# CMU-SAFARI/AirLift

Hardware: NVIDIA B200
Metric: remapped reads/sec at 1/2/4/8 B200; ksw2 GCUPS; seed-lookup HBM GB/s (higher is better)
Workload: dtype u8/int32

## Files before the change

airlift_b200/csrc/mmg_stages.cu:

```cuda
#include <cub/cub.cuh>
#include "mmg_ctx.cuh"
#include "mmg_regheap.h"
#include "mmg_sketchwarp.h"
#include "mmg_rswarp.h"

int mmg_run_sketch(mmg_ctx_t *c, const uint32_t *d_S, const SketchUnit *d_units, int n_units, int w, int k, int is_hpc,
                   DevBuf &cnt, DevBuf &off, DevBuf &out, int64_t *total, bool short_reads, uint64_t stage_slots);

#define MMG_READ_CHUNK 4096


__global__ void k_encode_reads(const uint8_t *__restrict__ ascii, const uint64_t *__restrict__ seq_off, const int32_t *__restrict__ seq_len,
                               const uint64_t *__restrict__ q_off, const uint8_t *__restrict__ flip, int n_seq, uint64_t n_words,
                               uint32_t *__restrict__ Q)
{
	const uint64_t wi = (uint64_t)blockIdx.x * blockDim.x + threadIdx.x;
	if (wi >= n_words) return;
	const uint64_t b0 = wi * 8;
	int lo = 0, hi = n_seq - 1;
	while (lo < hi) { const int mid = (lo + hi + 1) >> 1; if (q_off[mid] <= b0) lo = mid; else hi = mid - 1; }
	const int r = lo, len = seq_len[r];
	const uint64_t base = b0 - q_off[r];
	const uint8_t *s = ascii + seq_off[r];
	const bool fl = flip[r] != 0;
	uint32_t word = 0;
	for (int j = 0; j < 8; ++j) {
		const uint64_t i = base + j;
// ... 48 lines not shown
			if (n > 0 && n < max_occ) run += n;
		}
	}
	if (replay) {
		const int m = (int)(e - b);
		uint8_t dup = m > 256 ? 1 : 0;
		for (int i = 0; i < m && !dup; ++i) {
			if (m_n[b + i] <= 0 || m_n[b + i] >= max_occ) continue;
			const uint64_t h = mv[b + i].x >> 8;
			for (int j = i + 1; j < m; ++j)
				if (mv[b + j].x >> 8 == h && m_n[b + j] > 0 && m_n[b + j] < max_occ) { dup = 1; break; }
		}
		if (dup) {
			int kept = 0;
			for (int i = 0; i < m; ++i) kept += m_n[b + i] > 0 && m_n[b + i] < max_occ;
			dup = (kept <= 256 && n_a < (1 << 24)) ? 1 : 2;
		}
		replay[li] = dup;
	}
}

__global__ void k_expand(FragTab ft, const int32_t *__restrict__ list, int n_list, const mm128 *__restrict__ mv, const int32_t *__restrict__ m_n,
                         const uint64_t *__restrict__ m_val, const uint64_t *__restrict__ pos, int max_occ, int64_t flag,
                         const int64_t *__restrict__ aoff, const uint8_t *__restrict__ replay, int64_t n_total,
                         uint64_t *__restrict__ key, uint64_t *__restrict__ val, int32_t *__restrict__ n_skipped, const int32_t *__restrict__ m_aoff)
{
	const int64_t g = (int64_t)blockIdx.x * blockDim.x + threadIdx.x;
	if (g >= n_total) return;
	const int li = frag_of_anchor(aoff, n_list, g);
	if (replay[li] == 2) return;
	const int f = list ? list[li] : li;
	const int64_t b = ft.unit_off[ft.unit0[f]], e = ft.unit_off[ft.unit0[f + 1]];
	int64_t i = g - aoff[li];
	int m;
	{
		int lo = 0, hi = (int)(e - b) - 1;
		while (lo < hi) { const int mid = (lo + hi + 1) >> 1; if (m_aoff[b + mid] <= i) lo = mid; else hi = mid - 1; }
		m = lo;
		i -= m_aoff[b + m];
	}
	const mm128 mz = mv[b + m];
	const uint64_t r = mmg_hit_pos(pos, m_n[b + m], m_val[b + m], (uint32_t)i);
	if (replay[li] == 1) { key[g] = r, val[g] = (uint64_t)(g - aoff[li]); return; }
	if (mmg_skip_seed(flag, r, (uint32_t)mz.y)) { key[g] = MMG_NONE, val[g] = 0; atomicAdd(&n_skipped[li], 1); return; }
	const mm128 an = mmg_make_anchor(r, mz, mmg_is_tandem(mv + b, (int)(e - b), m), ft.qlen[f]);
	key[g] = (an.x & (1ULL << 63)) | r;
	val[g] = an.y;
}

__global__ void k_sort_segments(int n_list, const int64_t *__restrict__ aoff, const uint8_t *__restrict__ replay, int64_t *__restrict__ seg_b, int64_t *__restrict__ seg_e)
{
	const int li = blockIdx.x * blockDim.x + threadIdx.x;
	if (li >= n_list) return;
	seg_b[li] = aoff[li];
	seg_e[li] = replay[li] == 2 ? aoff[li] : aoff[li + 1];
}

__global__ void k_emit_sorted(int n_list, const int64_t *__restrict__ aoff, const uint8_t *__restrict__ replay, int64_t n_total,
                              const uint64_t *__restrict__ key, const uint64_t *__restrict__ val, const int32_t *__restrict__ n_skipped,
                              int32_t *__restrict__ na, mm128 *__restrict__ a, uint8_t *__restrict__ tie )
{
	const int64_t g = (int64_t)blockIdx.x * blockDim.x + threadIdx.x;
	if (g >= n_total) return;
	const int li = frag_of_anchor(aoff, n_list, g);
	if (replay[li]) return;
	const uint64_t k = key[g];
	if (g == aoff[li]) na[li] = (int32_t)(aoff[li + 1] - aoff[li]) - n_skipped[li];
	if (k == MMG_NONE) return;
	const uint64_t r = k & ~(1ULL << 63);
	mm128 an;
	an.x = (k & (1ULL << 63)) | (r & 0xffffffff00000000ULL) | ((uint32_t)r >> 1);
	an.y = val[g];
	a[g] = an;
	if (tie && g > aoff[li]) {
		const uint64_t kp = key[g - 1], rp = kp & ~(1ULL << 63);
		if (((kp & (1ULL << 63)) | (rp & 0xffffffff00000000ULL) | ((uint32_t)rp >> 1)) == an.x) tie[li] = 1;
	}
}

__global__ void __launch_bounds__(128)
k_fill_flat_warp(int n_list, const int64_t *__restrict__ aoff, const uint8_t *__restrict__ tie, const uint64_t *__restrict__ key,
                 const uint64_t *__restrict__ val, int32_t *__restrict__ na, mm128 *__restrict__ a, int32_t *__restrict__ work, RsFrame *__restrict__ stack)
{
	__shared__ int32_t s_head[4][256], s_tail[4][256];
	const int li = (int)(((int64_t)blockIdx.x * blockDim.x + threadIdx.x) >> 5), lane = threadIdx.x & 31, wi = threadIdx.x >> 5;
	if (li >= n_list || tie[li] != 1) return;
	const int64_t ao = aoff[li];
	const int32_t n_plan = (int32_t)(aoff[li + 1] - ao);
	mm128 *A = a + ao;
	int32_t o = 0;
	for (int32_t i0 = 0; i0 < n_plan; i0 += 32) {
		const int32_t i = i0 + lane;
		const uint64_t k = i < n_plan ? key[ao + i] : MMG_NONE;
		const unsigned m = __ballot_sync(0xffffffffu, k != MMG_NONE);
		if (k != MMG_NONE) {
			const uint64_t r = k & ~(1ULL << 63);
			mm128 an;
			an.x = (k & (1ULL << 63)) | (r & 0xffffffff00000000ULL) | ((uint32_t)r >> 1);
			an.y = val[ao + i];
			A[o + __popc(m & ((1u << lane) - 1u))] = an;
		}
		o += __popc(m);
	}
	__syncwarp();
	mm128 *tmp = reinterpret_cast<mm128*>(work + ao * 8);
	int32_t *dst = reinterpret_cast<int32_t*>(tmp + n_plan);
	uint8_t *dig = reinterpret_cast<uint8_t*>(dst + n_plan);
	const WarpDev wp = {lane};
	mmg_rs_sort_warp(wp, A, (int64_t)o, tmp, dst, dig, stack + ao / 65 + 2 * (int64_t)li, s_head[wi], s_tail[wi], KeyX());
	if (lane == 0) na[li] = o;
}


__global__ void k_heap_rank(int n_list, const int64_t *__restrict__ aoff, const uint8_t *__restrict__ replay, int64_t n_total,
                            const uint64_t *__restrict__ key, const uint64_t *__restrict__ val, uint32_t *__restrict__ K)
{
	const int64_t g = (int64_t)blockIdx.x * blockDim.x + threadIdx.x;
	if (g >= n_total) return;
	const int li = frag_of_anchor(aoff, n_list, g);
	if (replay[li] != 1) return;
	const int64_t ao = aoff[li];
	int64_t l = g;
	const uint64_t k = key[g];
	while (l > ao && key[l - 1] == k) --l;
	K[ao + (int64_t)val[g]] = (uint32_t)(l - ao);
}

__global__ void k_heap_list(int n_list, const uint8_t *__restrict__ replay, int32_t *__restrict__ out, int32_t *__restrict__ counters)
{
	const int li = blockIdx.x * blockDim.x + threadIdx.x;
	if (li >= n_list) return;
	if (replay[li] == 1) out[atomicAdd(&counters[0], 1)] = li;
	else if (replay[li] == 2) atomicAdd(&counters[2], 1);
}

#define HEAP_MAX_LISTS 256
#define HEAP_RING 16

struct HeapList { int32_t first, cnt, cur, m; };

__device__ __forceinline__ void heap_sift_root(uint32_t *l, uint32_t n, uint32_t tmp, uint32_t *root_out)
{
	uint32_t i = 0, root = tmp;
	const uint32_t INF = 0xffffffffu;
	for (;;) {
		const uint32_t c = 2 * i + 1;
		if (c >= n) break;
		const uint32_t g = 2 * c + 1;
		const uint32_t a = l[c], b = c + 1 < n ? l[c + 1] : INF;
		const uint32_t g0 = g < n ? l[g] : INF, g1 = g + 1 < n ? l[g + 1] : INF, g2 = g + 2 < n ? l[g + 2] : INF, g3 = g + 3 < n ? l[g + 3] : INF;
		const bool right = c + 1 < n && (a >> 8) > (b >> 8);
		const uint32_t k = right ? c + 1 : c, v = right ? b : a;
		if ((v >> 8) > (tmp >> 8)) break;
		l[i] = v;
		if (i == 0) root = v;
		i = k;
		const uint32_t c2 = 2 * k + 1;
// ... 1169 lines not shown
                    int64_t n_mv, int max_occ, const PassBufs &pb, bool want_mini, uint8_t *d_flag, int64_t *n_anchors)
{
	*n_anchors = 0;
	if (n_list == 0) return MMG_OK;
	MMG_TRY(pb.na->ensure((size_t)(n_list + 1) * 4));
	MMG_TRY(pb.aoff->ensure((size_t)(n_list + 1) * 8));
	MMG_TRY(pb.rep->ensure((size_t)(n_list + 1) * 4));
	MMG_TRY(pb.nmini->ensure((size_t)(n_list + 1) * 4));
	MMG_TRY(pb.nu->ensure((size_t)(n_list + 1) * 4));
	MMG_TRY(pb.nv->ensure((size_t)(n_list + 1) * 4));
	if (want_mini) MMG_TRY(pb.mini->ensure((size_t)(n_mv + 1) * 8));
	const bool heap_path = (opt->flag & MMG_F_HEAP_SORT) != 0;
	MMG_TRY(c->d_replay.ensure((size_t)n_list + 16));
	MMG_CUDA(cudaMemsetAsync(pb.na->p, 0, (size_t)(n_list + 1) * 4, c->stream));
	MMG_CUDA(cudaMemsetAsync(pb.nu->p, 0, (size_t)(n_list + 1) * 4, c->stream));
	MMG_CUDA(cudaMemsetAsync(pb.nv->p, 0, (size_t)(n_list + 1) * 4, c->stream));
	MMG_CUDA(cudaMemsetAsync(pb.nmini->p, 0, (size_t)(n_list + 1) * 4, c->stream));
	MMG_LAUNCH(c, k_plan, mmg_blocks(n_list, 128), 128, 0, ft, d_list, n_list, c->d_mv.as<mm128>(), c->d_m_n.as<int32_t>(), max_occ,
	           pb.na->as<int32_t>(), pb.rep->as<int32_t>(), pb.nmini->as<int32_t>(), want_mini ? pb.mini->as<uint64_t>() : nullptr,
	           heap_path ? c->d_replay.as<uint8_t>() : nullptr, c->d_m_aoff.as<int32_t>());
	MMG_TRY(scan_i32_to_i64(c, pb.na->as<int32_t>(), pb.aoff->as<int64_t>(), n_list + 1));
	int32_t *hp_counters = nullptr, *rlist = nullptr, *hp = nullptr;
	if (heap_path) {
		MMG_TRY(c->d_hlist.ensure(((size_t)n_list + 8) * 4));
		MMG_TRY(c->h_path.ensure(64));
		hp_counters = c->d_hlist.as<int32_t>(), rlist = hp_counters + 4, hp = c->h_path.as<int32_t>() + (d_flag ? 0 : 4);
		MMG_CUDA(cudaMemsetAsync(hp_counters, 0, 16, c->stream));
		MMG_LAUNCH(c, k_heap_list, mmg_blocks(n_list, 256), 256, 0, n_list, c->d_replay.as<uint8_t>(), rlist, hp_counters);
		MMG_D2H(c, hp, hp_counters, 16);
	}
	int64_t tot = 0;
	MMG_D2H(c, &tot, pb.aoff->as<int64_t>() + n_list, 8);
	MMG_CUDA(cudaStreamSynchronize(c->stream));
	*n_anchors = tot;
	MMG_TRY(pb.a->ensure((size_t)(tot + 1) * 16));
	MMG_TRY(pb.work->ensure((size_t)(tot + 1) * 32));
	MMG_TRY(pb.u->ensure((size_t)(tot + 1) * 16));
	MMG_TRY(pb.b->ensure((size_t)(tot + 1) * 16));
	MMG_TRY(pb.stack->ensure((size_t)(tot / 65 + 2 * (size_t)n_list + 4) * sizeof(RsFrame)));
	MMG_TRY(c->d_heap.ensure((size_t)(n_mv + 1) * 16));
	uint8_t *d_tie = nullptr;
	if (!heap_path) {
		MMG_TRY(c->d_tie.ensure((size_t)n_list + 16));
		d_tie = c->d_tie.as<uint8_t>();
		MMG_CUDA(cudaMemsetAsync(d_tie, 0, (size_t)n_list + 16, c->stream));
		MMG_CUDA(cudaMemsetAsync(c->d_replay.p, 0, (size_t)n_list + 16, c->stream));
	}
	if (tot > 0) {
		MMG_TRY(c->d_skey.ensure(((size_t)tot + 1) * 16)); MMG_TRY(c->d_sval.ensure(((size_t)tot + 1) * 16));
		MMG_TRY(c->d_sseg.ensure(((size_t)n_list + 1) * 20 + 64));
		uint64_t *k0 = c->d_skey.as<uint64_t>(), *k1 = k0 + tot + 1, *v0 = c->d_sval.as<uint64_t>(), *v1 = v0 + tot + 1;
		int64_t *seg_b = c->d_sseg.as<int64_t>(), *seg_e = seg_b + n_list + 1;
		int32_t *n_skipped = reinterpret_cast<int32_t*>(seg_e + n_list + 1);
		MMG_CUDA(cudaMemsetAsync(n_skipped, 0, (size_t)n_list * 4, c->stream));
		MMG_LAUNCH(c, k_expand, mmg_blocks(tot, 256), 256, 0, ft, d_list, n_list, c->d_mv.as<mm128>(), c->d_m_n.as<int32_t>(), c->d_m_val.as<uint64_t>(),
		           mi->d_pos, max_occ, opt->flag, pb.aoff->as<int64_t>(), c->d_replay.as<uint8_t>(), tot, k0, v0, n_skipped, c->d_m_aoff.as<int32_t>());
		MMG_LAUNCH(c, k_sort_segments, mmg_blocks(n_list, 256), 256, 0, n_list, pb.aoff->as<int64_t>(), c->d_replay.as<uint8_t>(), seg_b, seg_e);
		{
			size_t tmp = 0;
			cub::DeviceSegmentedSort::SortPairs(nullptr, tmp, k0, k1, v0, v1, tot, n_list, seg_b, seg_e, c->stream);
			MMG_TRY(c->d_cub.ensure(tmp));
			MMG_TIMED(c, "cub_segmented_sort(seed hits)", cub::DeviceSegmentedSort::SortPairs(c->d_cub.p, tmp, k0, k1, v0, v1, tot, n_list, seg_b, seg_e, c->stream));
		}
		MMG_LAUNCH(c, k_emit_sorted, mmg_blocks(tot, 256), 256, 0, n_list, pb.aoff->as<int64_t>(), c->d_replay.as<uint8_t>(), tot, k1, v1, n_skipped,
		           pb.na->as<int32_t>(), pb.a->as<mm128>(), d_tie);
	}
	if (heap_path && tot > 0) {
		MMG_TRY(c->d_hrank.ensure(((size_t)tot + 1) * 4));
		MMG_TRY(c->d_hpop.ensure(((size_t)tot + 1) * 4));
		int32_t *counters = hp_counters;
		const uint64_t *k1 = c->d_skey.as<uint64_t>() + tot + 1, *v1 = c->d_sval.as<uint64_t>() + tot + 1;
		if (hp[0] > 0) {
			MMG_LAUNCH(c, k_heap_rank, mmg_blocks(tot, 256), 256, 0, n_list, pb.aoff->as<int64_t>(), c->d_replay.as<uint8_t>(), tot, k1, v1, c->d_hrank.as<uint32_t>());
			MMG_LAUNCH(c, k_heap_replay, hp[0] < 148 * 8 ? hp[0] : 148 * 8, 32, 0, ft, d_list, rlist, counters, c->d_mv.as<mm128>(), c->d_m_n.as<int32_t>(), c->d_m_val.as<uint64_t>(),
			           c->d_m_aoff.as<int32_t>(), mi->d_pos, max_occ, opt->flag, pb.aoff->as<int64_t>(), c->d_hrank.as<uint32_t>(), c->d_hpop.as<uint32_t>());
			MMG_LAUNCH(c, k_heap_emit, hp[0], HEAP_EMIT_THREADS, 0, ft, d_list, rlist, c->d_mv.as<mm128>(), c->d_m_n.as<int32_t>(), c->d_m_val.as<uint64_t>(),
			           c->d_m_aoff.as<int32_t>(), mi->d_pos, max_occ, opt->flag, pb.aoff->as<int64_t>(), c->d_hpop.as<uint32_t>(), pb.na->as<int32_t>(), pb.a->as<mm128>(),
			           c->d_frag_iter.as<unsigned long long>() + 1);
		}
	}
	if (!heap_path) {
		if (tot > 0)
			MMG_LAUNCH(c, k_fill_flat_warp, mmg_blocks((size_t)n_list * 32, 128), 128, 0, n_list, pb.aoff->as<int64_t>(), d_tie, c->d_skey.as<uint64_t>(),
			           c->d_sval.as<uint64_t>(), pb.na->as<int32_t>(), pb.a->as<mm128>(), pb.work->as<int32_t>(), pb.stack->as<RsFrame>());
	} else {
		const int per_warp = d_flag == nullptr || n_list <= 4096 ? 1 : 0;
		MMG_LAUNCH(c, k_fill, mmg_blocks(per_warp ? (size_t)n_list * 32 : (size_t)n_list, 64), 64, 0, ft, d_list, n_list, c->d_mv.as<mm128>(), c->d_m_n.as<int32_t>(),
		           c->d_m_val.as<uint64_t>(), mi->d_pos, max_occ, opt->flag, pb.aoff->as<int64_t>(), pb.na->as<int32_t>(), pb.a->as<mm128>(), c->d_heap.as<mm128>(),
		           pb.stack->as<RsFrame>(), heap_path ? c->d_replay.as<uint8_t>() : d_tie, heap_path ? 2 : 1, per_warp);
	}
	if (getenv("MMG_TRACE")) {
		std::vector<uint8_t> hr((size_t)n_list); std::vector<int32_t> hn((size_t)n_list);
		cudaStreamSynchronize(c->stream);
		cudaMemcpy(hr.data(), heap_path ? c->d_replay.p : (void*)d_tie, (size_t)n_list, cudaMemcpyDeviceToHost);
		cudaMemcpy(hn.data(), pb.na->p, (size_t)n_list * 4, cudaMemcpyDeviceToHost);
		int64_t nr = 0, ar = 0, amax = 0, big = 0, abig = 0, big_all = 0, abig_all = 0;
		for (int i = 0; i < n_list; ++i) {
			if (hn[i] > 4096) ++big_all, abig_all += hn[i];
			if (!hr[i]) continue;
			++nr, ar += hn[i]; if (hn[i] > amax) amax = hn[i]; if (hn[i] > 4096) ++big, abig += hn[i];
		}
		fprintf(stderr, "[mmg::pass] max_occ %d: %d fragments, %lld anchors; > 4096 anchors: %lld fragments with %lld anchors; literal replay: %lld fragments, %lld anchors, largest %lld, "
		        "of which > 4096 anchors: %lld fragments with %lld anchors\n", max_occ, n_list, (long long)tot, (long long)big_all, (long long)abig_all, (long long)nr, (long long)ar, (long long)amax, (long long)big, (long long)abig);
	}
	ChainOptDev co;
	co.bw = opt->bw, co.max_gap = opt->max_gap, co.max_gap_ref = opt->max_gap_ref, co.max_frag_len = opt->max_frag_len;
	co.max_skip = opt->max_chain_skip, co.max_iter = opt->max_chain_iter, co.min_cnt = opt->min_cnt, co.min_sc = opt->min_chain_score;
	co.is_cdna = !!(opt->flag & MMG_F_SPLICE), co.is_sr = !!(opt->flag & MMG_F_SR);
	if (tot > 0) {
		MMG_TRY(c->d_seg_head.ensure((size_t)tot + 16));
		MMG_TRY(c->d_seg_start.ensure(((size_t)tot + 2) * 8 + 64));
		MMG_TRY(c->d_seg_avg.ensure((size_t)(n_list + 1) * 4));
		int64_t *seg_start = c->d_seg_start.as<int64_t>();
		int32_t *d_nseg = reinterpret_cast<int32_t*>(seg_start + tot + 1), *d_next = d_nseg + 1, *d_nlong = d_nseg + 2;
		MMG_CUDA(cudaMemsetAsync(d_nseg, 0, 16, c->stream));
		MMG_TRY(c->d_seg_li.ensure(((size_t)tot + 1) * 4));
		MMG_TRY(c->d_seg_long.ensure(((size_t)tot / CHAIN_SMALL_SEG + 2) * 4));
		MMG_LAUNCH(c, k_chain_heads, mmg_blocks(tot, 256), 256, 0, ft, d_list, n_list, c->d_misc.as<int32_t>(), co, pb.aoff->as<int64_t>(),
		           pb.na->as<int32_t>(), pb.a->as<mm128>(), tot, c->d_seg_head.as<uint8_t>(), pb.work->as<int32_t>(), c->d_seg_li.as<int32_t>());
		MMG_LAUNCH(c, k_chain_avgspan, mmg_blocks((size_t)n_list * 32, 128), 128, 0, n_list, pb.aoff->as<int64_t>(), pb.na->as<int32_t>(),
		           pb.a->as<mm128>(), c->d_seg_avg.as<float>());
		{
			size_t tmp = 0;
			cub::CountingInputIterator<int64_t> it(0);
			cub::DeviceSelect::Flagged(nullptr, tmp, it, c->d_seg_head.as<uint8_t>(), seg_start, d_nseg, tot, c->stream);
			MMG_TRY(c->d_cub.ensure(tmp));
// ... 51 lines not shown
{
	MMG_CUDA(cudaSetDevice(c->dev));
	ResidentBatch &rb = c->rb;
	const int nf = rb.n_frag;
	memset(out, 0, sizeof(*out));
	out->n_frag = nf;
	if (nf == 0) return MMG_OK;
	if (mi->w > MMG_MAX_W) { mmg_set_error("w=%d exceeds the device limit %d", mi->w, MMG_MAX_W); return MMG_ELIMIT; }
	MMG_CUDA(cudaEventRecord(c->ev[0], c->stream));
	int64_t n_mv = 0;
	MMG_TRY(mmg_run_sketch(c, c->d_Q.as<uint32_t>(), c->d_units.as<SketchUnit>(), rb.n_units, mi->w, mi->k, mi->is_hpc, c->d_unit_cnt,
	                       c->d_unit_off, c->d_mv, &n_mv, rb.max_len <= SKW_MAX_LEN, rb.q_words * 8));
	MMG_TRY(c->d_m_n.ensure((size_t)(n_mv + 1) * 4));
	MMG_TRY(c->d_m_val.ensure((size_t)(n_mv + 1) * 8));
	MMG_TRY(c->d_m_aoff.ensure((size_t)(n_mv + 1) * 4));
	if (n_mv) MMG_LAUNCH(c, k_lookup, mmg_blocks(n_mv, 256), 256, 0, mi->view(), c->d_mv.as<mm128>(), n_mv, c->d_m_n.as<int32_t>(), c->d_m_val.as<uint64_t>());
	FragTab ft;
	ft.unit0 = c->d_frag_unit0.as<int32_t>(), ft.unit_off = c->d_unit_off.as<int64_t>(), ft.qlen = c->d_frag_qlen.as<int32_t>();
	const bool want_mini = !(opt->flag & MMG_F_SR);
	MMG_TRY(c->d_frag_flag.ensure((size_t)nf + 16));
	MMG_TRY(c->d_frag_iter.ensure(16));
	MMG_CUDA(cudaMemsetAsync(c->d_frag_flag.p, 0, (size_t)nf + 16, c->stream));
	MMG_CUDA(cudaMemsetAsync(c->d_frag_iter.p, 0, 16, c->stream));
	MMG_TRY(c->h_path.ensure(64));
	memset(c->h_path.p, 0, 64);
	PassBufs p1 = {&c->d_frag_na, &c->d_frag_aoff, &c->d_frag_rep, &c->d_frag_nmini, &c->d_mini, &c->d_a, &c->d_work, &c->d_u, &c->d_b,
	               &c->d_stack, &c->d_frag_nu, &c->d_frag_nv};
	int64_t n_anch1 = 0, n_anch2 = 0;
	MMG_TRY(run_pass(c, mi, opt, ft, nullptr, nf, n_mv, opt->mid_occ, p1, want_mini, c->d_frag_flag.as<uint8_t>(), &n_anch1));
	std::vector<int32_t> list;
	std::vector<uint8_t> hflag(nf);
	MMG_TRY(c->d_frag_list.ensure((size_t)(nf + 1) * 8));
	int32_t *d_list = c->d_frag_list.as<int32_t>(), *d_src = d_list + nf;
	MMG_CUDA(cudaMemsetAsync(d_src, 0xff, (size_t)nf * 4, c->stream));
	if (opt->max_occ > opt->mid_occ) {
		MMG_D2H(c, hflag.data(), c->d_frag_flag.p, nf);
		MMG_CUDA(cudaStreamSynchronize(c->stream));
		for (int f = 0; f < nf; ++f) if (hflag[f]) list.push_back(f);
	}
	PassBufs p2 = {&c->d2_frag_na, &c->d2_frag_aoff, &c->d2_frag_rep, &c->d2_frag_nmini, &c->d2_mini, &c->d2_a, &c->d2_work, &c->d2_u, &c->d2_b,
	               &c->d2_stack, &c->d2_frag_nu, &c->d2_frag_nv};
	const int n2 = (int)list.size();
	if (n2) {
		MMG_H2D(c, d_list, list.data(), (size_t)n2 * 4);
		MMG_TRY(run_pass(c, mi, opt, ft, d_list, n2, n_mv, opt->max_occ, p2, want_mini, nullptr, &n_anch2));
		MMG_LAUNCH(c, k_merge_pass2, mmg_blocks(n2, 128), 128, 0, n2, d_list, c->d2_frag_nu.as<int32_t>(), c->d2_frag_nv.as<int32_t>(),
		           c->d2_frag_rep.as<int32_t>(), c->d2_frag_nmini.as<int32_t>(), c->d_frag_nu.as<int32_t>(), c->d_frag_nv.as<int32_t>(),
		           c->d_frag_rep.as<int32_t>(), c->d_frag_nmini.as<int32_t>(), d_src);
// ... 34 lines not shown
		uint64_t *ho = reinterpret_cast<uint64_t*>(c->h_out_meta.as<uint8_t>() + ((meta_i + 15) & ~(size_t)15));
		MMG_D2H(c, hi, c->d_frag_nu.p, (size_t)nf * 4);
		MMG_D2H(c, hi + nf, c->d_frag_nv.p, (size_t)nf * 4);
		MMG_D2H(c, hi + 2 * nf, c->d_frag_rep.p, (size_t)nf * 4);
		MMG_D2H(c, hi + 3 * nf, c->d_frag_nmini.p, (size_t)nf * 4);
		MMG_D2H(c, hi + 4 * nf, d_src, (size_t)nf * 4);
		MMG_D2H(c, ho, c->d_uoff.p, (size_t)(nf + 1) * 8);
		MMG_D2H(c, ho + (nf + 1), c->d_voff.p, (size_t)(nf + 1) * 8);
		if (want_mini) MMG_D2H(c, ho + 2 * (nf + 1), c->d_moff.p, (size_t)(nf + 1) * 8);
		if (tot[0]) MMG_D2H(c, c->h_out_u.p, c->d_out_u.p, (size_t)tot[0] * 8);
		if (tot[1]) MMG_D2H(c, c->h_out_a.p, c->d_out_a.p, (size_t)tot[1] * 16);
		if (tot[2]) MMG_D2H(c, c->h_out_mini.p, c->d_out_mini.p, (size_t)tot[2] * 8);
		MMG_CUDA(cudaEventRecord(c->ev[2], c->stream));
		MMG_CUDA(cudaStreamSynchronize(c->stream));
		for (int f = 0; f < nf; ++f) hi[4 * nf + f] = hi[4 * nf + f] >= 0 ? 1 : 0;
		if (!want_mini) { for (int f = 0; f < nf; ++f) hi[3 * nf + f] = 0; memset(ho + 2 * (nf + 1), 0, (size_t)(nf + 1) * 8); }
		out->n_u = hi, out->n_a = hi + nf, out->rep_len = hi + 2 * nf, out->n_mini = hi + 3 * nf, out->rechained = hi + 4 * nf;
		out->u_off = ho, out->a_off = ho + (nf + 1), out->mini_off = ho + 2 * (nf + 1);
		out->u = c->h_out_u.as<uint64_t>(), out->a = c->h_out_a.as<mmg128_t>(), out->mini_pos = c->h_out_mini.as<uint64_t>();
		float ms = 0;
		cudaEventElapsedTime(&ms, c->ev[1], c->ev[2]); out->t_d2h_ms = ms;
	} else MMG_CUDA(cudaStreamSynchronize(c->stream));
	{
		const int32_t *hp = c->h_path.as<int32_t>();
		c->path[0] += (uint64_t)n2, c->path[1] += (uint64_t)(hp[0] + hp[4]), c->path[2] += (uint64_t)(hp[2] + hp[6]);
		c->path[6] += c->h_path.as<unsigned long long>()[5];
	}
	float ms = 0;
	cudaEventElapsedTime(&ms, c->ev[0], c->ev[1]); out->t_kernels_ms = ms;
	out->n_chain_iter = iters;
	return MMG_OK;
}

extern "C" int mmg_seed_chain_batch(mmg_ctx_t *c, const mmg_idx_t *mi, const mmg_mapopt_t *opt, const mmg_batch_t *b, mmg_chains_t *out)
{
	MMG_CUDA(cudaSetDevice(c->dev));
	MMG_CUDA(cudaEventRecord(c->ev[3], c->stream));
	MMG_TRY(mmg_batch_upload(c, opt, b));
	MMG_TRY(mmg_seed_chain_resident(c, mi, opt, out, 1));
	float ms = 0;
	cudaEventElapsedTime(&ms, c->ev[3], c->ev[0]); out->t_h2d_ms = ms;
	return MMG_OK;
}


extern "C" int mmg_sketch(mmg_ctx_t *c, const char *str, int len, int w, int k, uint32_t rid, int is_hpc, mmg128_t *out, int cap, int *n_out)
{
	*n_out = 0;
// ... 102 lines not shown
```

Baseline: 7.034 million.

## Replace CUB segmented sort in heap path with size-classed in-kernel seed ordering

In the heap path, seed hits are no longer expanded globally and sorted with cub::DeviceSegmentedSort. Fragments are now classified by hit count into warp, CTA and big classes. Each class generates keys on the fly, bitonic-sorts tiles in shared memory, and for big fragments runs multi-pass merge-path merges through global scratch. Ranks for literal-replay fragments and anchors for normal fragments are emitted directly, removing the expand/sort/emit/rank kernels and their global key/value traffic. The cost is more complex code, several extra launches per merge round for big fragments, and heavy shared-memory use.

```diff
diff --git a/airlift_b200/csrc/mmg_seedorder.h b/airlift_b200/csrc/mmg_seedorder.h
--- /dev/null
+++ b/airlift_b200/csrc/mmg_seedorder.h
@@ -0,0 +1,141 @@
+#ifndef MMG_SEEDORDER_H
+#define MMG_SEEDORDER_H
+#include "mmg_core.h"
+
+template <int N> struct GroupEmu {
+	static constexpr int NT = N;
+	template <class F> void each(F &&f) const { for (int t = 0; t < N; ++t) f(t); }
+	static void aadd(int32_t *p, int32_t v) { *p += v; }
+};
+#ifdef __CUDACC__
+template <int N> struct GroupDev {
+	static constexpr int NT = N;
+	int t;
+	template <class F> __device__ void each(F &&f) const { f(t); if (N == 32) __syncwarp(); else __syncthreads(); }
+	static __device__ void aadd(int32_t *p, int32_t v) { atomicAdd(p, v); }
+};
+#endif
+
+MMG_HD int32_t so_corank(const uint64_t *A, int32_t la, const uint64_t *B, int32_t lb, int32_t d)
+{
+	int32_t lo = d > lb ? d - lb : 0, hi = d < la ? d : la;
+	while (lo < hi) { const int32_t mid = (lo + hi) >> 1; if (A[mid] <= B[d - 1 - mid]) lo = mid + 1; else hi = mid; }
+	return lo;
+}
+
+template <class G>
+MMG_HDN inline void so_bitonic(const G &g, uint64_t *k, uint32_t *v, int32_t n)
+{
+	for (int32_t size = 2; size <= n; size <<= 1)
+		for (int32_t j = size >> 1; j > 0; j >>= 1)
+			g.each([&](int t) {
+				for (int32_t i = t; i < n >> 1; i += G::NT) {
+					const int32_t lo = ((i & ~(j - 1)) << 1) | (i & (j - 1)), hi = lo + j;
+					const bool up = (lo & size) == 0;
+					const uint64_t a = k[lo], b = k[hi];
+					if ((a > b) == up) { k[lo] = b, k[hi] = a; const uint32_t x = v[lo]; v[lo] = v[hi], v[hi] = x; }
+				}
+			});
+}
+
+template <class G, int TILE, class KeyOf>
+MMG_HDN inline void so_chunk(const G &g, int32_t c0, int32_t len, KeyOf key_of, uint64_t *sk, uint32_t *sv, int32_t *s_kept)
+{
+	int32_t np = 2;
+	while (np < len) np <<= 1;
+	g.each([&](int t) {
+		int32_t kept = 0;
+		for (int32_t i = t; i < np; i += G::NT) {
+			uint64_t k = MMG_NONE; uint32_t v = 0xffffffffu;
+			if (i < len) { v = (uint32_t)(c0 + i); k = key_of(v); kept += k != MMG_NONE; }
+			sk[i] = k, sv[i] = v;
+		}
+		if (kept) G::aadd(s_kept, kept);
+	});
+	so_bitonic(g, sk, sv, np);
+}
+
+struct SoTile { int32_t ps, la, lb, d0, d1; };
+template <int TILE>
+MMG_HD SoTile so_tile(int32_t n, int64_t w, int32_t tile)
+{
+	SoTile T;
+	const int64_t o = (int64_t)tile * TILE;
+	T.ps = (int32_t)(o / (2 * w) * (2 * w));
+	T.la = (int32_t)(n - T.ps < w ? n - T.ps : w);
+	T.lb = (int32_t)(n - T.ps - w <= 0 ? 0 : n - T.ps - w < w ? n - T.ps - w : w);
+	T.d0 = (int32_t)(o - T.ps);
+	T.d1 = T.d0 + TILE < T.la + T.lb ? T.d0 + TILE : T.la + T.lb;
+	return T;
+}
+
+template <class G, int TILE>
+MMG_HDN inline void so_merge_tile(const G &g, const SoTile &T, int64_t w, int32_t i0, int32_t i1, const uint64_t *ak, const uint32_t *av,
+                                  uint64_t *bk, uint32_t *bv, uint64_t *sk, uint32_t *sv)
+{
+	constexpr int NT = G::NT, IPT = TILE / NT;
+	const int32_t j0 = T.d0 - i0, j1 = T.d1 - i1, na = i1 - i0, nb = j1 - j0;
+	g.each([&](int t) {
+		for (int32_t x = t; x < na + nb; x += NT) {
+			const int64_t src = x < na ? (int64_t)T.ps + i0 + x : (int64_t)T.ps + w + j0 + (x - na);
+			sk[x] = ak[src], sv[x] = av[src];
+		}
+	});
+	g.each([&](int t) {
+		const int32_t dd = t * IPT;
+		if (dd >= na + nb) return;
+		int32_t ia = so_corank(sk, na, sk + na, nb, dd), ib = dd - ia;
+		for (int q = 0; q < IPT && dd + q < na + nb; ++q) {
+			const bool take_a = ib >= nb || (ia < na && sk[ia] <= sk[na + ib]);
+			const int32_t s = take_a ? ia++ : na + ib++;
+			bk[T.ps + T.d0 + dd + q] = sk[s], bv[T.ps + T.d0 + dd + q] = sv[s];
+		}
+	});
+}
+
+template <class Emit>
+MMG_HD void so_emit_one(const uint64_t *k, const uint32_t *v, int32_t i, Emit &emit)
+{
+	int32_t f = i;
+	if (k[i] != MMG_NONE) while (f > 0 && k[f - 1] == k[i]) --f;
+	emit(i, k[i], v[i], f);
+}
+
+template <class G, int TILE, class KeyOf, class Emit>
+MMG_HDN inline int32_t mmg_seed_order(const G &g, int32_t n, KeyOf key_of, uint64_t *sk, uint32_t *sv, int32_t *s_w,
+                                      uint64_t *gk0, uint32_t *gv0, uint64_t *gk1, uint32_t *gv1, Emit emit)
+{
+	constexpr int NT = G::NT, IPT = TILE / NT;
+	static_assert(IPT * NT == TILE && (TILE & (TILE - 1)) == 0, "TILE: a power of two and a multiple of the group");
+	g.each([&](int t) { if (t == 0) s_w[0] = 0; });
+	for (int32_t c0 = 0; c0 < n; c0 += TILE) {
+		const int32_t len = n - c0 < TILE ? n - c0 : TILE;
+		so_chunk<G, TILE>(g, c0, len, key_of, sk, sv, &s_w[0]);
+		if (n > TILE) g.each([&](int t) { for (int32_t i = t; i < len; i += NT) gk0[c0 + i] = sk[i], gv0[c0 + i] = sv[i]; });
+	}
+	const int32_t kept = s_w[0];
+	if (n <= TILE) {
+		g.each([&](int t) { for (int32_t i = t; i < n; i += NT) so_emit_one(sk, sv, i, emit); });
+		return kept;
+	}
+	uint64_t *ak = gk0, *bk = gk1; uint32_t *av = gv0, *bv = gv1;
+	const int32_t n_tiles = (n + TILE - 1) / TILE;
+	for (int64_t w = TILE; w < n; w <<= 1) {
+		for (int32_t g0 = 0; g0 < n_tiles; g0 += NT) {
+			g.each([&](int t) {
+				if (g0 + t >= n_tiles) return;
+				const SoTile T = so_tile<TILE>(n, w, g0 + t);
+				s_w[1 + t] = so_corank(ak + T.ps, T.la, ak + T.ps + w, T.lb, T.d0);
+				s_w[1 + NT + t] = so_corank(ak + T.ps, T.la, ak + T.ps + w, T.lb, T.d1);
+			});
+			const int32_t g1 = g0 + NT < n_tiles ? g0 + NT : n_tiles;
+			for (int32_t tile = g0; tile < g1; ++tile)
+				so_merge_tile<G, TILE>(g, so_tile<TILE>(n, w, tile), w, s_w[1 + tile - g0], s_w[1 + NT + tile - g0], ak, av, bk, bv, sk, sv);
+		}
+		uint64_t *tk = ak; ak = bk, bk = tk;
+		uint32_t *tv = av; av = bv, bv = tv;
+	}
+	g.each([&](int t) { for (int32_t i = t; i < n; i += NT) so_emit_one(ak, av, i, emit); });
+	return kept;
+}
+#endif
diff --git a/airlift_b200/csrc/mmg_stages.cu b/airlift_b200/csrc/mmg_stages.cu
--- a/airlift_b200/csrc/mmg_stages.cu
+++ b/airlift_b200/csrc/mmg_stages.cu
@@ -3,6 +3,7 @@
 #include "mmg_regheap.h"
 #include "mmg_sketchwarp.h"
 #include "mmg_rswarp.h"
+#include "mmg_seedorder.h"
 
 int mmg_run_sketch(mmg_ctx_t *c, const uint32_t *d_S, const SketchUnit *d_units, int n_units, int w, int k, int is_hpc,
                    DevBuf &cnt, DevBuf &off, DevBuf &out, int64_t *total, bool short_reads, uint64_t stage_slots);
@@ -97,13 +98,12 @@
 
 __global__ void k_expand(FragTab ft, const int32_t *__restrict__ list, int n_list, const mm128 *__restrict__ mv, const int32_t *__restrict__ m_n,
                          const uint64_t *__restrict__ m_val, const uint64_t *__restrict__ pos, int max_occ, int64_t flag,
-                         const int64_t *__restrict__ aoff, const uint8_t *__restrict__ replay, int64_t n_total,
+                         const int64_t *__restrict__ aoff, int64_t n_total,
                          uint64_t *__restrict__ key, uint64_t *__restrict__ val, int32_t *__restrict__ n_skipped, const int32_t *__restrict__ m_aoff)
 {
 	const int64_t g = (int64_t)blockIdx.x * blockDim.x + threadIdx.x;
 	if (g >= n_total) return;
 	const int li = frag_of_anchor(aoff, n_list, g);
-	if (replay[li] == 2) return;
 	const int f = list ? list[li] : li;
 	const int64_t b = ft.unit_off[ft.unit0[f]], e = ft.unit_off[ft.unit0[f + 1]];
 	int64_t i = g - aoff[li];
@@ -116,29 +116,19 @@
 	}
 	const mm128 mz = mv[b + m];
 	const uint64_t r = mmg_hit_pos(pos, m_n[b + m], m_val[b + m], (uint32_t)i);
-	if (replay[li] == 1) { key[g] = r, val[g] = (uint64_t)(g - aoff[li]); return; }
 	if (mmg_skip_seed(flag, r, (uint32_t)mz.y)) { key[g] = MMG_NONE, val[g] = 0; atomicAdd(&n_skipped[li], 1); return; }
 	const mm128 an = mmg_make_anchor(r, mz, mmg_is_tandem(mv + b, (int)(e - b), m), ft.qlen[f]);
 	key[g] = (an.x & (1ULL << 63)) | r;
 	val[g] = an.y;
 }
 
-__global__ void k_sort_segments(int n_list, const int64_t *__restrict__ aoff, const uint8_t *__restrict__ replay, int64_t *__restrict__ seg_b, int64_t *__restrict__ seg_e)
-{
-	const int li = blockIdx.x * blockDim.x + threadIdx.x;
-	if (li >= n_list) return;
-	seg_b[li] = aoff[li];
-	seg_e[li] = replay[li] == 2 ? aoff[li] : aoff[li + 1];
-}
-
-__global__ void k_emit_sorted(int n_list, const int64_t *__restrict__ aoff, const uint8_t *__restrict__ replay, int64_t n_total,
+__global__ void k_emit_sorted(int n_list, const int64_t *__restrict__ aoff, int64_t n_total,
                               const uint64_t *__restrict__ key, const uint64_t *__restrict__ val, const int32_t *__restrict__ n_skipped,
-                              int32_t *__restrict__ na, mm128 *__restrict__ a, uint8_t *__restrict__ tie )
+                              int32_t *__restrict__ na, mm128 *__restrict__ a, uint8_t *__restrict__ tie)
 {
 	const int64_t g = (int64_t)blockIdx.x * blockDim.x + threadIdx.x;
 	if (g >= n_total) return;
 	const int li = frag_of_anchor(aoff, n_list, g);
-	if (replay[li]) return;
 	const uint64_t k = key[g];
 	if (g == aoff[li]) na[li] = (int32_t)(aoff[li + 1] - aoff[li]) - n_skipped[li];
 	if (k == MMG_NONE) return;
@@ -147,7 +137,7 @@
 	an.x = (k & (1ULL << 63)) | (r & 0xffffffff00000000ULL) | ((uint32_t)r >> 1);
 	an.y = val[g];
 	a[g] = an;
-	if (tie && g > aoff[li]) {
+	if (g > aoff[li]) {
 		const uint64_t kp = key[g - 1], rp = kp & ~(1ULL << 63);
 		if (((kp & (1ULL << 63)) | (rp & 0xffffffff00000000ULL) | ((uint32_t)rp >> 1)) == an.x) tie[li] = 1;
 	}
@@ -186,28 +176,214 @@
 	if (lane == 0) na[li] = o;
 }
 
-
-__global__ void k_heap_rank(int n_list, const int64_t *__restrict__ aoff, const uint8_t *__restrict__ replay, int64_t n_total,
-                            const uint64_t *__restrict__ key, const uint64_t *__restrict__ val, uint32_t *__restrict__ K)
-{
-	const int64_t g = (int64_t)blockIdx.x * blockDim.x + threadIdx.x;
-	if (g >= n_total) return;
-	const int li = frag_of_anchor(aoff, n_list, g);
-	if (replay[li] != 1) return;
-	const int64_t ao = aoff[li];
-	int64_t l = g;
-	const uint64_t k = key[g];
-	while (l > ao && key[l - 1] == k) --l;
-	K[ao + (int64_t)val[g]] = (uint32_t)(l - ao);
-}
-
-__global__ void k_heap_list(int n_list, const uint8_t *__restrict__ replay, int32_t *__restrict__ out, int32_t *__restrict__ counters)
-{
-	const int li = blockIdx.x * blockDim.x + threadIdx.x;
-	if (li >= n_list) return;
-	if (replay[li] == 1) out[atomicAdd(&counters[0], 1)] = li;
-	else if (replay[li] == 2) atomicAdd(&counters[2], 1);
-}
+#define SO_LISTS 256
+#define SO_WARP_MAX 256
+#define SO_CTA_MAX 2048
+#define SO_BIG_TILE 8192
+#define SO_BIG_NT 512
+
+template <int NT, int TILE>
+struct SoSmem { uint64_t k[TILE]; uint32_t v[TILE]; int32_t first[SO_LISTS], m[SO_LISTS], w[2 * NT + 1], n_lists; };
+
+struct SoArgs {
+	FragTab ft; const int32_t *list; const mm128 *mv; const int32_t *m_n; const uint64_t *m_val; const int32_t *m_aoff; const uint64_t *pos;
+	int max_occ; int64_t flag; const int64_t *aoff; const uint8_t *replay; int32_t *na; mm128 *a; uint32_t *K; int32_t *work;
+};
+
+struct SoFrag {
+	const SoArgs *A; const int32_t *first, *m;
+	int64_t b, ao; int32_t n; int n_mv, qlen, n_lists; bool ranks;
+	__device__ int list_of(uint32_t slot) const {
+		int lo = 0, hi = n_lists - 1;
+		while (lo < hi) { const int mid = (lo + hi + 1) >> 1; if ((uint32_t)first[mid] <= slot) lo = mid; else hi = mid - 1; }
+		return lo;
+	}
+	__device__ uint64_t key(uint32_t slot) const {
+		const int j = list_of(slot), mm = m[j];
+		const uint64_t r = mmg_hit_pos(A->pos, A->m_n[b + mm], A->m_val[b + mm], slot - (uint32_t)first[j]);
+		if (ranks) return r;
+		const uint32_t qp = (uint32_t)A->mv[b + mm].y;
+		if (mmg_skip_seed(A->flag, r, qp)) return MMG_NONE;
+		return ((r & 1) != (qp & 1) ? 1ULL << 63 : 0) | r;
+	}
+	__device__ void emit(int32_t k, uint64_t key, uint32_t slot, int32_t first_eq) const {
+		if (ranks) { A->K[ao + slot] = (uint32_t)first_eq; return; }
+		if (key == MMG_NONE) return;
+		const int mm = m[list_of(slot)];
+		A->a[ao + k] = mmg_make_anchor(key & ~(1ULL << 63), A->mv[b + mm], mmg_is_tandem(A->mv + b, n_mv, mm), qlen);
+	}
+	__device__ uint64_t *gk(int i) const { return reinterpret_cast<uint64_t*>(A->work + ao * 8) + (size_t)i * n; }
+	__device__ uint32_t *gv(int i) const { return reinterpret_cast<uint32_t*>(gk(2)) + (size_t)i * n; }
+};
+
+template <int NT, int TILE>
+__device__ __forceinline__ SoFrag so_frag(int t, int li, const SoArgs &A, SoSmem<NT, TILE> &S)
+{
+	const unsigned FULL = 0xffffffffu;
+	SoFrag F;
+	const int f = A.list ? A.list[li] : li;
+	const int64_t e = A.ft.unit_off[A.ft.unit0[f + 1]];
+	F.A = &A, F.first = S.first, F.m = S.m;
+	F.b = A.ft.unit_off[A.ft.unit0[f]], F.ao = A.aoff[li], F.n = (int32_t)(A.aoff[li + 1] - F.ao);
+	F.n_mv = (int)(e - F.b), F.qlen = A.ft.qlen[f], F.ranks = A.replay[li] == 1;
+	if (t < 32) {
+		int n_lists = 0;
+		for (int i0 = 0; i0 < F.n_mv; i0 += 32) {
+			const int i = i0 + t;
+			const bool kept = i < F.n_mv && A.m_n[F.b + i] > 0 && A.m_n[F.b + i] < A.max_occ;
+			const unsigned mk = __ballot_sync(FULL, kept);
+			if (kept) { const int j = n_lists + __popc(mk & ((1u << t) - 1u)); S.first[j] = A.m_aoff[F.b + i], S.m[j] = i; }
+			n_lists += __popc(mk);
+		}
+		if (t == 0) S.n_lists = n_lists, S.w[0] = 0;
+	}
+	if (NT == 32) __syncwarp(); else __syncthreads();
+	F.n_lists = S.n_lists;
+	return F;
+}
+
+template <int NT, int TILE>
+__device__ __forceinline__ void seed_order_frag(const GroupDev<NT> &g, SoSmem<NT, TILE> &S, int li, const SoArgs &A)
+{
+	const SoFrag F = so_frag<NT, TILE>(g.t, li, A, S);
+	auto key_of = [&](uint32_t slot) { return F.key(slot); };
+	auto emit = [&](int32_t k, uint64_t key, uint32_t slot, int32_t first) { F.emit(k, key, slot, first); };
+	const int32_t kept = mmg_seed_order<GroupDev<NT>, TILE>(g, F.n, key_of, S.k, S.v, S.w, F.gk(0), F.gv(0), F.gk(1), F.gv(1), emit);
+	if (!F.ranks && g.t == 0) A.na[li] = kept;
+}
+
+__global__ void __launch_bounds__(128) k_seed_order_warp(SoArgs A, const int32_t *__restrict__ olist, int n_work)
+{
+	__shared__ SoSmem<32, SO_WARP_MAX> s[4];
+	const int wi = threadIdx.x >> 5, w = blockIdx.x * 4 + wi;
+	if (w >= n_work) return;
+	seed_order_frag<32, SO_WARP_MAX>(GroupDev<32>{(int)(threadIdx.x & 31)}, s[wi], olist[w], A);
+}
+
+__global__ void __launch_bounds__(256) k_seed_order_cta(SoArgs A, const int32_t *__restrict__ olist)
+{
+	__shared__ SoSmem<256, SO_CTA_MAX> s;
+	seed_order_frag<256, SO_CTA_MAX>(GroupDev<256>{(int)threadIdx.x}, s, olist[blockIdx.x], A);
+}
+
+typedef SoSmem<SO_BIG_NT, SO_BIG_TILE> SoBigSmem;
+
+__device__ __forceinline__ bool so_big_tile(const int64_t *tile_off, int n_big, int *fi, int32_t *tile)
+{
+	const int64_t t = blockIdx.x;
+	if (t >= tile_off[n_big]) return false;
+	int lo = 0, hi = n_big - 1;
+	while (lo < hi) { const int mid = (lo + hi + 1) >> 1; if (tile_off[mid] <= t) lo = mid; else hi = mid - 1; }
+	*fi = lo, *tile = (int32_t)(t - tile_off[lo]);
+	return true;
+}
+
+__device__ __forceinline__ int so_big_rounds(int32_t n) { int r = 0; while (((int64_t)SO_BIG_TILE << r) < n) ++r; return r; }
+
+__global__ void __launch_bounds__(SO_BIG_NT) k_seed_big_chunk(SoArgs A, const int32_t *__restrict__ big, const int64_t *__restrict__ tile_off, int n_big)
+{
+	extern __shared__ __align__(16) unsigned char so_smem[];
+	SoBigSmem &S = *reinterpret_cast<SoBigSmem*>(so_smem);
+	int fi; int32_t tile;
+	if (!so_big_tile(tile_off, n_big, &fi, &tile)) return;
+	const int li = big[fi], t = threadIdx.x;
+	const SoFrag F = so_frag<SO_BIG_NT, SO_BIG_TILE>(t, li, A, S);
+	const GroupDev<SO_BIG_NT> g = {t};
+	const int32_t c0 = tile * SO_BIG_TILE, len = F.n - c0 < SO_BIG_TILE ? F.n - c0 : SO_BIG_TILE;
+	so_chunk<GroupDev<SO_BIG_NT>, SO_BIG_TILE>(g, c0, len, [&](uint32_t slot) { return F.key(slot); }, S.k, S.v, &S.w[0]);
+	if (F.n <= SO_BIG_TILE) {
+		for (int32_t i = t; i < F.n; i += SO_BIG_NT) {
+			auto emit = [&](int32_t k, uint64_t key, uint32_t slot, int32_t first) { F.emit(k, key, slot, first); };
+			so_emit_one(S.k, S.v, i, emit);
+		}
+		if (!F.ranks && t == 0) A.na[li] = S.w[0];
+		return;
+	}
+	uint64_t *gk = F.gk(0); uint32_t *gv = F.gv(0);
+	for (int32_t i = t; i < len; i += SO_BIG_NT) gk[c0 + i] = S.k[i], gv[c0 + i] = S.v[i];
+}
+
+__device__ __forceinline__ int32_t so_corank_warp(const uint64_t *A, int32_t la, const uint64_t *B, int32_t lb, int32_t d, int lane)
+{
+	int32_t lo = d > lb ? d - lb : 0, hi = d < la ? d : la;
+	while (lo < hi) {
+		const int32_t stride = (hi - lo + 31) >> 5, x = lo + lane * stride;
+		const bool p = x < hi && A[x] <= B[d - 1 - x];
+		const int c = __popc(__ballot_sync(0xffffffffu, p));
+		const int32_t nlo = c ? lo + (c - 1) * stride + 1 : lo, nhi = lo + c * stride < hi ? lo + c * stride : hi;
+		lo = nlo, hi = nhi;
+	}
+	return lo;
+}
+
+__global__ void __launch_bounds__(SO_BIG_NT) k_seed_big_merge(SoArgs A, const int32_t *__restrict__ big, const int64_t *__restrict__ tile_off, int n_big, int r)
+{
+	extern __shared__ __align__(16) unsigned char so_smem[];
+	SoBigSmem &S = *reinterpret_cast<SoBigSmem*>(so_smem);
+	int fi; int32_t tile;
+	if (!so_big_tile(tile_off, n_big, &fi, &tile)) return;
+	const int li = big[fi], t = threadIdx.x;
+	const int64_t ao = A.aoff[li], w = (int64_t)SO_BIG_TILE << r;
+	const int32_t n = (int32_t)(A.aoff[li + 1] - ao);
+	if (w >= n) return;
+	SoFrag F; F.A = &A, F.ao = ao, F.n = n;
+	const uint64_t *ak = F.gk(r & 1); const uint32_t *av = F.gv(r & 1);
+	const SoTile T = so_tile<SO_BIG_TILE>(n, w, tile);
+	if (t < 64) {
+		const int32_t i = so_corank_warp(ak + T.ps, T.la, ak + T.ps + w, T.lb, t < 32 ? T.d0 : T.d1, t & 31);
+		if ((t & 31) == 0) S.w[1 + (t >> 5)] = i;
+	}
+	__syncthreads();
+	so_merge_tile<GroupDev<SO_BIG_NT>, SO_BIG_TILE>(GroupDev<SO_BIG_NT>{t}, T, w, S.w[1], S.w[2], ak, av, F.gk((r + 1) & 1), F.gv((r + 1) & 1), S.k, S.v);
+}
+
+__global__ void __launch_bounds__(SO_BIG_NT) k_seed_big_emit(SoArgs A, const int32_t *__restrict__ big, const int64_t *__restrict__ tile_off, int n_big)
+{
+	extern __shared__ __align__(16) unsigned char so_smem[];
+	SoBigSmem &S = *reinterpret_cast<SoBigSmem*>(so_smem);
+	int fi; int32_t tile;
+	if (!so_big_tile(tile_off, n_big, &fi, &tile)) return;
+	const int li = big[fi], t = threadIdx.x;
+	const int32_t n = (int32_t)(A.aoff[li + 1] - A.aoff[li]);
+	if (n <= SO_BIG_TILE) return;
+	const SoFrag F = so_frag<SO_BIG_NT, SO_BIG_TILE>(t, li, A, S);
+	const int R = so_big_rounds(n);
+	const uint64_t *k = F.gk(R & 1); const uint32_t *v = F.gv(R & 1);
+	const int32_t i1 = (tile + 1) * SO_BIG_TILE < n ? (tile + 1) * SO_BIG_TILE : n;
+	auto emit = [&](int32_t kk, uint64_t key, uint32_t slot, int32_t first) { F.emit(kk, key, slot, first); };
+	for (int32_t i = tile * SO_BIG_TILE + t; i < i1; i += SO_BIG_NT) {
+		so_emit_one(k, v, i, emit);
+		if (!F.ranks) {
+			if (k[i] != MMG_NONE && (i + 1 == n || k[i + 1] == MMG_NONE)) A.na[li] = i + 1;
+			else if (i == 0 && k[0] == MMG_NONE) A.na[li] = 0;
+		}
+	}
+}
+
+__global__ void k_seed_classes(int n_list, const uint8_t *__restrict__ replay, const int64_t *__restrict__ aoff, int32_t *__restrict__ counters,
+                               int32_t *__restrict__ rlist, int32_t *__restrict__ cls, int32_t *__restrict__ big_tiles)
+{
+	const unsigned FULL = 0xffffffffu;
+	const int li = blockIdx.x * blockDim.x + threadIdx.x, lane = threadIdx.x & 31;
+	const int r = li < n_list ? replay[li] : 2;
+	if (r == 1) rlist[atomicAdd(&counters[0], 1)] = li;
+	else if (r == 2 && li < n_list) atomicAdd(&counters[2], 1);
+	const int64_t n = r != 2 ? aoff[li + 1] - aoff[li] : 0;
+	const int c = n == 0 ? -1 : n <= SO_WARP_MAX ? 0 : n <= SO_CTA_MAX ? 1 : 2;
+	for (int cc = 0; cc < 3; ++cc) {
+		const unsigned mk = __ballot_sync(FULL, c == cc);
+		if (!mk) continue;
+		int base = 0;
+		if (lane == __ffs(mk) - 1) base = atomicAdd(&counters[4 + cc], __popc(mk));
+		base = __shfl_sync(FULL, base, __ffs(mk) - 1);
+		if (c == cc) {
+			const int at = base + __popc(mk & ((1u << lane) - 1u));
+			cls[(size_t)cc * n_list + at] = li;
+			if (cc == 2) big_tiles[at] = (int32_t)((n + SO_BIG_TILE - 1) / SO_BIG_TILE), atomicMax(&counters[7], (int32_t)n);
+		}
+	}
+}
+
 
 #define HEAP_MAX_LISTS 256
 #define HEAP_RING 16
@@ -1423,12 +1599,13 @@
 	MMG_TRY(scan_i32_to_i64(c, pb.na->as<int32_t>(), pb.aoff->as<int64_t>(), n_list + 1));
 	int32_t *hp_counters = nullptr, *rlist = nullptr, *hp = nullptr;
 	if (heap_path) {
-		MMG_TRY(c->d_hlist.ensure(((size_t)n_list + 8) * 4));
-		MMG_TRY(c->h_path.ensure(64));
-		hp_counters = c->d_hlist.as<int32_t>(), rlist = hp_counters + 4, hp = c->h_path.as<int32_t>() + (d_flag ? 0 : 4);
-		MMG_CUDA(cudaMemsetAsync(hp_counters, 0, 16, c->stream));
-		MMG_LAUNCH(c, k_heap_list, mmg_blocks(n_list, 256), 256, 0, n_list, c->d_replay.as<uint8_t>(), rlist, hp_counters);
-		MMG_D2H(c, hp, hp_counters, 16);
+		MMG_TRY(c->d_hlist.ensure(((size_t)n_list * 8 + 16) * 4));
+		MMG_TRY(c->h_path.ensure(128));
+		hp_counters = c->d_hlist.as<int32_t>(), rlist = hp_counters + 8, hp = c->h_path.as<int32_t>() + 16 + (d_flag ? 0 : 8);
+		MMG_CUDA(cudaMemsetAsync(hp_counters, 0, 32, c->stream));
+		MMG_LAUNCH(c, k_seed_classes, mmg_blocks(n_list, 256), 256, 0, n_list, c->d_replay.as<uint8_t>(), pb.aoff->as<int64_t>(), hp_counters, rlist,
+		           rlist + n_list, rlist + 4 * (size_t)n_list);
+		MMG_D2H(c, hp, hp_counters, 32);
 	}
 	int64_t tot = 0;
 	MMG_D2H(c, &tot, pb.aoff->as<int64_t>() + n_list, 8);
@@ -1445,35 +1622,54 @@
 		MMG_TRY(c->d_tie.ensure((size_t)n_list + 16));
 		d_tie = c->d_tie.as<uint8_t>();
 		MMG_CUDA(cudaMemsetAsync(d_tie, 0, (size_t)n_list + 16, c->stream));
-		MMG_CUDA(cudaMemsetAsync(c->d_replay.p, 0, (size_t)n_list + 16, c->stream));
-	}
-	if (tot > 0) {
+	}
+	if (!heap_path && tot > 0) {
 		MMG_TRY(c->d_skey.ensure(((size_t)tot + 1) * 16)); MMG_TRY(c->d_sval.ensure(((size_t)tot + 1) * 16));
-		MMG_TRY(c->d_sseg.ensure(((size_t)n_list + 1) * 20 + 64));
+		MMG_TRY(c->d_sseg.ensure(((size_t)n_list + 1) * 4 + 64));
 		uint64_t *k0 = c->d_skey.as<uint64_t>(), *k1 = k0 + tot + 1, *v0 = c->d_sval.as<uint64_t>(), *v1 = v0 + tot + 1;
-		int64_t *seg_b = c->d_sseg.as<int64_t>(), *seg_e = seg_b + n_list + 1;
-		int32_t *n_skipped = reinterpret_cast<int32_t*>(seg_e + n_list + 1);
+		int32_t *n_skipped = c->d_sseg.as<int32_t>();
+		const int64_t *seg = pb.aoff->as<int64_t>();
 		MMG_CUDA(cudaMemsetAsync(n_skipped, 0, (size_t)n_list * 4, c->stream));
 		MMG_LAUNCH(c, k_expand, mmg_blocks(tot, 256), 256, 0, ft, d_list, n_list, c->d_mv.as<mm128>(), c->d_m_n.as<int32_t>(), c->d_m_val.as<uint64_t>(),
-		           mi->d_pos, max_occ, opt->flag, pb.aoff->as<int64_t>(), c->d_replay.as<uint8_t>(), tot, k0, v0, n_skipped, c->d_m_aoff.as<int32_t>());
-		MMG_LAUNCH(c, k_sort_segments, mmg_blocks(n_list, 256), 256, 0, n_list, pb.aoff->as<int64_t>(), c->d_replay.as<uint8_t>(), seg_b, seg_e);
+		           mi->d_pos, max_occ, opt->flag, seg, tot, k0, v0, n_skipped, c->d_m_aoff.as<int32_t>());
 		{
 			size_t tmp = 0;
-			cub::DeviceSegmentedSort::SortPairs(nullptr, tmp, k0, k1, v0, v1, tot, n_list, seg_b, seg_e, c->stream);
+			cub::DeviceSegmentedSort::SortPairs(nullptr, tmp, k0, k1, v0, v1, tot, n_list, seg, seg + 1, c->stream);
 			MMG_TRY(c->d_cub.ensure(tmp));
-			MMG_TIMED(c, "cub_segmented_sort(seed hits)", cub::DeviceSegmentedSort::SortPairs(c->d_cub.p, tmp, k0, k1, v0, v1, tot, n_list, seg_b, seg_e, c->stream));
-		}
-		MMG_LAUNCH(c, k_emit_sorted, mmg_blocks(tot, 256), 256, 0, n_list, pb.aoff->as<int64_t>(), c->d_replay.as<uint8_t>(), tot, k1, v1, n_skipped,
-		           pb.na->as<int32_t>(), pb.a->as<mm128>(), d_tie);
+			MMG_TIMED(c, "cub_segmented_sort(seed hits)", cub::DeviceSegmentedSort::SortPairs(c->d_cub.p, tmp, k0, k1, v0, v1, tot, n_list, seg, seg + 1, c->stream));
+		}
+		MMG_LAUNCH(c, k_emit_sorted, mmg_blocks(tot, 256), 256, 0, n_list, seg, tot, k1, v1, n_skipped, pb.na->as<int32_t>(), pb.a->as<mm128>(), d_tie);
 	}
 	if (heap_path && tot > 0) {
 		MMG_TRY(c->d_hrank.ensure(((size_t)tot + 1) * 4));
 		MMG_TRY(c->d_hpop.ensure(((size_t)tot + 1) * 4));
-		int32_t *counters = hp_counters;
-		const uint64_t *k1 = c->d_skey.as<uint64_t>() + tot + 1, *v1 = c->d_sval.as<uint64_t>() + tot + 1;
+		int32_t *cls = rlist + n_list, *big = cls + 2 * (size_t)n_list, *big_tiles = rlist + 4 * (size_t)n_list;
+		int64_t *tile_off = reinterpret_cast<int64_t*>(rlist + 6 * (size_t)n_list + 2);
+		const int n_big = hp[6];
+		SoArgs sa = {ft, d_list, c->d_mv.as<mm128>(), c->d_m_n.as<int32_t>(), c->d_m_val.as<uint64_t>(), c->d_m_aoff.as<int32_t>(), mi->d_pos, max_occ,
+		             opt->flag, pb.aoff->as<int64_t>(), c->d_replay.as<uint8_t>(), pb.na->as<int32_t>(), pb.a->as<mm128>(), c->d_hrank.as<uint32_t>(),
+		             pb.work->as<int32_t>()};
+		if (n_big) {
+			static bool attr_set = false;
+			if (!attr_set) {
+				MMG_CUDA(cudaFuncSetAttribute(k_seed_big_chunk, cudaFuncAttributeMaxDynamicSharedMemorySize, (int)sizeof(SoBigSmem)));
+				MMG_CUDA(cudaFuncSetAttribute(k_seed_big_merge, cudaFuncAttributeMaxDynamicSharedMemorySize, (int)sizeof(SoBigSmem)));
+				MMG_CUDA(cudaFuncSetAttribute(k_seed_big_emit, cudaFuncAttributeMaxDynamicSharedMemorySize, (int)sizeof(SoBigSmem)));
+				attr_set = true;
+			}
+			MMG_CUDA(cudaMemsetAsync(big_tiles + n_big, 0, 4, c->stream));
+			MMG_TRY(scan_i32_to_i64(c, big_tiles, tile_off, n_big + 1));
+			const unsigned grid = (unsigned)(tot / SO_BIG_TILE + n_big + 1);
+			int rounds = 0;
+			while (((int64_t)SO_BIG_TILE << rounds) < hp[7]) ++rounds;
+			MMG_LAUNCH(c, k_seed_big_chunk, grid, SO_BIG_NT, sizeof(SoBigSmem), sa, big, tile_off, n_big);
+			for (int r = 0; r < rounds; ++r) MMG_LAUNCH(c, k_seed_big_merge, grid, SO_BIG_NT, sizeof(SoBigSmem), sa, big, tile_off, n_big, r);
+			if (rounds) MMG_LAUNCH(c, k_seed_big_emit, grid, SO_BIG_NT, sizeof(SoBigSmem), sa, big, tile_off, n_big);
+		}
+		if (hp[5]) MMG_LAUNCH(c, k_seed_order_cta, hp[5], 256, 0, sa, cls + n_list);
+		if (hp[4]) MMG_LAUNCH(c, k_seed_order_warp, mmg_blocks(hp[4], 4), 128, 0, sa, cls, hp[4]);
 		if (hp[0] > 0) {
-			MMG_LAUNCH(c, k_heap_rank, mmg_blocks(tot, 256), 256, 0, n_list, pb.aoff->as<int64_t>(), c->d_replay.as<uint8_t>(), tot, k1, v1, c->d_hrank.as<uint32_t>());
-			MMG_LAUNCH(c, k_heap_replay, hp[0] < 148 * 8 ? hp[0] : 148 * 8, 32, 0, ft, d_list, rlist, counters, c->d_mv.as<mm128>(), c->d_m_n.as<int32_t>(), c->d_m_val.as<uint64_t>(),
+			MMG_LAUNCH(c, k_heap_replay, hp[0] < 148 * 8 ? hp[0] : 148 * 8, 32, 0, ft, d_list, rlist, hp_counters, c->d_mv.as<mm128>(), c->d_m_n.as<int32_t>(), c->d_m_val.as<uint64_t>(),
 			           c->d_m_aoff.as<int32_t>(), mi->d_pos, max_occ, opt->flag, pb.aoff->as<int64_t>(), c->d_hrank.as<uint32_t>(), c->d_hpop.as<uint32_t>());
 			MMG_LAUNCH(c, k_heap_emit, hp[0], HEAP_EMIT_THREADS, 0, ft, d_list, rlist, c->d_mv.as<mm128>(), c->d_m_n.as<int32_t>(), c->d_m_val.as<uint64_t>(),
 			           c->d_m_aoff.as<int32_t>(), mi->d_pos, max_occ, opt->flag, pb.aoff->as<int64_t>(), c->d_hpop.as<uint32_t>(), pb.na->as<int32_t>(), pb.a->as<mm128>(),
@@ -1503,6 +1699,16 @@
 		}
 		fprintf(stderr, "[mmg::pass] max_occ %d: %d fragments, %lld anchors; > 4096 anchors: %lld fragments with %lld anchors; literal replay: %lld fragments, %lld anchors, largest %lld, "
 		        "of which > 4096 anchors: %lld fragments with %lld anchors\n", max_occ, n_list, (long long)tot, (long long)big_all, (long long)abig_all, (long long)nr, (long long)ar, (long long)amax, (long long)big, (long long)abig);
+		if (heap_path) {
+			std::vector<int64_t> ha((size_t)n_list + 1);
+			cudaMemcpy(ha.data(), pb.aoff->p, ((size_t)n_list + 1) * 8, cudaMemcpyDeviceToHost);
+			int64_t hist[34] = {0};
+			for (int i = 0; i < n_list; ++i) if (hr[i] != 2 && ha[i + 1] > ha[i]) ++hist[64 - __builtin_clzll((unsigned long long)(ha[i + 1] - ha[i] - 1) | 1)];
+			fprintf(stderr, "[mmg::pass] max_occ %d: seed order: %d warp (<= %d hits), %d cta (<= %d), %d big (largest %d); fragments with <= 2^k planned hits:",
+			        max_occ, hp[4], SO_WARP_MAX, hp[5], SO_CTA_MAX, hp[6], hp[7]);
+			for (int k = 0; k < 34; ++k) if (hist[k]) fprintf(stderr, " 2^%d:%lld", k, (long long)hist[k]);
+			fprintf(stderr, "\n");
+		}
 	}
 	ChainOptDev co;
 	co.bw = opt->bw, co.max_gap = opt->max_gap, co.max_gap_ref = opt->max_gap_ref, co.max_frag_len = opt->max_frag_len;
@@ -1600,8 +1806,8 @@
 	MMG_TRY(c->d_frag_iter.ensure(16));
 	MMG_CUDA(cudaMemsetAsync(c->d_frag_flag.p, 0, (size_t)nf + 16, c->stream));
 	MMG_CUDA(cudaMemsetAsync(c->d_frag_iter.p, 0, 16, c->stream));
-	MMG_TRY(c->h_path.ensure(64));
-	memset(c->h_path.p, 0, 64);
+	MMG_TRY(c->h_path.ensure(128));
+	memset(c->h_path.p, 0, 128);
 	PassBufs p1 = {&c->d_frag_na, &c->d_frag_aoff, &c->d_frag_rep, &c->d_frag_nmini, &c->d_mini, &c->d_a, &c->d_work, &c->d_u, &c->d_b,
 	               &c->d_stack, &c->d_frag_nu, &c->d_frag_nv};
 	int64_t n_anch1 = 0, n_anch2 = 0;
@@ -1682,8 +1888,8 @@
 		cudaEventElapsedTime(&ms, c->ev[1], c->ev[2]); out->t_d2h_ms = ms;
 	} else MMG_CUDA(cudaStreamSynchronize(c->stream));
 	{
-		const int32_t *hp = c->h_path.as<int32_t>();
-		c->path[0] += (uint64_t)n2, c->path[1] += (uint64_t)(hp[0] + hp[4]), c->path[2] += (uint64_t)(hp[2] + hp[6]);
+		const int32_t *hp = c->h_path.as<int32_t>() + 16;
+		c->path[0] += (uint64_t)n2, c->path[1] += (uint64_t)(hp[0] + hp[8]), c->path[2] += (uint64_t)(hp[2] + hp[10]);
 		c->path[6] += c->h_path.as<unsigned long long>()[5];
 	}
 	float ms = 0;
```

Measured after the change: 7.252 million, median of 6. 1.03x the previous value.
